# mouzzarr/go-libp2p-pubsub

Measured on AMD Instinct MI355X. Metric: peer-heartbeat updates/sec + msg-edge deliveries/sec, 1M-peer gossipsub sim, higher is better.
Workload: dtype f64; 1 GPU; c3: 1000000 peers, random-regular k=32, one IP per peer, 16 topics, beacon-style params, 4 msg/s/topic, 10 rounds/heartbeat; peers_per_gpu=1000000, degree=32, topics=16, edge_topic_records=512000000, rounds_per_heartbeat=10

## Files before the change

go-libp2p-pubsub_amd/csrc/gsim_internal.h:

```cpp
#pragma once
#include <hip/hip_runtime.h>

#include <cstdint>
#include <string>
#include <vector>

#include "gsim.h"

#include <atomic>
namespace gsim {
extern std::atomic<unsigned long long> g_host_syncs;
inline hipError_t counted_stream_sync(hipStream_t s)
{
    g_host_syncs.fetch_add(1, std::memory_order_relaxed);
    return (hipStreamSynchronize)(s);
}
inline hipError_t counted_memcpy(void* dst, const void* src, size_t n, hipMemcpyKind k)
{
    g_host_syncs.fetch_add(1, std::memory_order_relaxed);
    return (hipMemcpy)(dst, src, n, k);
}
}
#define hipStreamSynchronize(s) ::gsim::counted_stream_sync(s)
#define hipMemcpy(d, s, n, k) ::gsim::counted_memcpy(d, s, n, k)
// ... 80 lines not shown
    return d > 0 ? div_trunc_pos(n, d) : n / d;
}

template <class A>
__device__ __forceinline__ const A& kernarg0(const A& arg)
{
    using CP = const __attribute__((address_space(4))) A*;
    CP p = (CP)__builtin_amdgcn_kernarg_segment_ptr();
    asm volatile("" : "+s"(p));
#ifdef GSIM_DEBUG_KERNARG
    static_assert(sizeof(A) >= 16, "kernarg0 check reads 16 bytes");
    const uint64_t* x = (const uint64_t*)&arg;
    const __attribute__((address_space(4))) uint64_t* y = (const __attribute__((address_space(4))) uint64_t*)p;
    if (x[0] != y[0] || x[1] != y[1]) __builtin_trap();
#else
    (void)arg;
#endif
    return *(const A*)p;
}

__device__ __forceinline__ int64_t lazy_mtime(int32_t lazy, int64_t R, int64_t graft, int64_t stored)
{
    return lazy && graft <= R ? R - graft : stored;
}

__device__ __forceinline__ uint64_t smask_of(const uint64_t* smask, uint32_t owner)
{
    return smask ? smask[owner] : ~0ull;
}
__device__ __forceinline__ bool slot_has(uint64_t m, int32_t t) { return (m >> t) & 1ull; }
__device__ __forceinline__ int64_t slot_idx(uint64_t m, int32_t t, int64_t E, int64_t x)
{
    return (int64_t)__popcll(m & ((1ull << t) - 1ull)) * E + x;
}
__device__ __forceinline__ int32_t slot_topic(uint64_t m, int32_t p)
{
    for (int32_t k = 0; k < p; ++k) m &= m - 1;
    return m ? __builtin_ctzll(m) : -1;
}

typedef const __attribute__((address_space(4))) gsim_topic_score_params* ctp_t;
__device__ __forceinline__ ctp_t const_tp(const gsim_topic_score_params* p)
{
    return (ctp_t)(p);
}

enum FieldKind : int {
    FK_RAW = 0,
    FK_RECORD,
    FK_TRECORD,
    FK_TEDGE,
    FK_TFLAGS,
    FK_ESTATE,
    FK_SEEN,
};

struct FieldRef {
    void* ptr;
    size_t bytes;
    int kind = FK_RAW;
    int elem = 1;
    int npar = 1;
};

struct Deliver;

// ... 411 lines not shown
```

go-libp2p-pubsub_amd/csrc/heartbeat.hip:

```cpp
#include <hip/hip_runtime.h>

#include <algorithm>
#include <vector>

#include "gsim.h"
#include "gsim_internal.h"
#include "philox.h"

using namespace gsim;

constexpr int kGiantRow = 8192;
constexpr int kWideB = 1024;
constexpr int kWideBytes = 64;
#ifndef GSIM_HB_HUBV
#define GSIM_HB_HUBV 2
#endif
#define GSIM_HUB_SCHEME_(s1, s2, s3) (GSIM_HB_HUBV == 1 ? (s1) : GSIM_HB_HUBV == 2 ? (s2) : (s3))
constexpr int kHubB[6] = {GSIM_HUB_SCHEME_(128, 64, 64), GSIM_HUB_SCHEME_(256, 128, 64), GSIM_HUB_SCHEME_(512, 256, 128),
                          GSIM_HUB_SCHEME_(1024, 512, 256), 1024, 1024};
constexpr int kHubVv[6] = {GSIM_HUB_SCHEME_(1, 2, 2), GSIM_HUB_SCHEME_(1, 2, 4), GSIM_HUB_SCHEME_(1, 2, 4),
                           GSIM_HUB_SCHEME_(1, 2, 4), 2, 4};
static_assert(kHubB[0] * kHubVv[0] == 128 && kHubB[1] * kHubVv[1] == 256 && kHubB[2] * kHubVv[2] == 512 &&
              kHubB[3] * kHubVv[3] == 1024 && kHubB[4] * kHubVv[4] == 2048 && kHubB[5] * kHubVv[5] == 4096,
              "a hub class's block covers its longest row");

struct Extra {
    uint8_t* d_ctl = nullptr;
    uint64_t* d_cany = nullptr;
    int64_t* d_lastpub = nullptr;
    uint64_t* d_fantopics = nullptr;
    uint32_t max_degree = 0;
    uint64_t seed = 0x9E3779B97F4A7C15ull;
    uint32_t* d_rows = nullptr;
    int64_t n16 = 0, n32 = 0, n64 = 0;
    int64_t n8 = 0;
// ... 120 lines not shown
    if constexpr (W == 64) {
        return wave_min_u32(v);
    } else {
        static_assert(W == 32 || W == 16 || W == 8, "groups of 8, 16, 32 or 64 lanes");
        const int I = -1;
        v = min(v, (uint32_t)__builtin_amdgcn_update_dpp(I, (int)v, 0x111, 0xF, 0xF, false));
        v = min(v, (uint32_t)__builtin_amdgcn_update_dpp(I, (int)v, 0x112, 0xF, 0xF, false));
        v = min(v, (uint32_t)__builtin_amdgcn_update_dpp(I, (int)v, 0x114, 0xF, 0xF, false));
        if constexpr (W == 8) {
            uint32_t r = 0;
#pragma unroll
            for (int q = 0; q < 8; ++q) {
                const uint32_t x = (uint32_t)__builtin_amdgcn_readlane((int)v, 8 * q + 7);
                if (grp == q) r = x;
            }
            return r;
        }
        v = min(v, (uint32_t)__builtin_amdgcn_update_dpp(I, (int)v, 0x118, 0xF, 0xF, false));
        if constexpr (W == 32) {
            v = min(v, (uint32_t)__builtin_amdgcn_update_dpp(I, (int)v, 0x142, 0xA, 0xF, false));
            const uint32_t lo = (uint32_t)__builtin_amdgcn_readlane((int)v, 31);
            const uint32_t hi = (uint32_t)__builtin_amdgcn_readlane((int)v, 63);
            return grp ? hi : lo;
        } else {
            const uint32_t r0 = (uint32_t)__builtin_amdgcn_readlane((int)v, 15);
            const uint32_t r1 = (uint32_t)__builtin_amdgcn_readlane((int)v, 31);
            const uint32_t r2 = (uint32_t)__builtin_amdgcn_readlane((int)v, 47);
            const uint32_t r3 = (uint32_t)__builtin_amdgcn_readlane((int)v, 63);
            return grp == 0 ? r0 : grp == 1 ? r1 : grp == 2 ? r2 : r3;
        }
    }
}

__device__ __forceinline__ uint32_t glob(const HbArgs& a, uint32_t p) { return a.gid ? a.gid[p] : p; }

__device__ __forceinline__ uint64_t hb_key(const HbArgs& a, uint32_t obs, int32_t t, uint32_t purpose, uint32_t col,
                                           uint32_t pos)
{
    return select_key(a.seed, (uint32_t)a.tick, obs, (uint32_t)t, purpose, col, pos);
}

__device__ __forceinline__ uint32_t hb_key_hi(const HbArgs& a, uint32_t obs, int32_t t, uint32_t purpose,
                                              uint32_t col, uint32_t pos)
{
    return (uint32_t)(select_key(a.seed, (uint32_t)a.tick, obs, (uint32_t)t, purpose, col, pos) >> 32);
}

template <int W = 64>
__device__ bool select_smallest(const HbArgs& a, bool cand, int count, uint32_t obs, int32_t t, uint32_t purpose,
                                uint32_t col, uint32_t pos, uint64_t gm = ~0ull, int grp = 0)
{
    const uint64_t avail = __ballot(cand) & gm;
    const int n = __popcll(avail);
    if (n == 0) return false;
    if (count <= 0 || n <= count) return cand;
    const int lane = threadIdx.x & 63;
    uint32_t hi = 0xFFFFFFFFu;
    if (cand) hi = hb_key_hi(a, obs, t, purpose, col, pos);
    const uint32_t tau = (uint32_t)((float)count / (float)n * 4294967040.0f);
    bool sel = cand && hi < tau;
    int c = __popcll(__ballot(sel) & gm);
    while (c > count) {
        const uint32_t mx = ~group_min_u32<W>(sel ? ~hi : 0xFFFFFFFFu, grp);
        const uint64_t at = __ballot(sel && hi == mx) & gm;
        const int win = 63 - __clzll((long long)at);
        if (lane == win) sel = false;
        --c;
    }
    uint32_t rest = (cand && !sel) ? hi : 0xFFFFFFFFu;
    uint64_t left = __ballot(cand && !sel) & gm;
    while (c < count) {
        const uint32_t mn = group_min_u32<W>(rest, grp);
        const int win = __ffsll((long long)(__ballot(rest == mn) & left)) - 1;
        left &= ~(1ull << win);
        if (lane == win) { sel = true; rest = 0xFFFFFFFFu; }
        ++c;
    }
    return sel;
}

__device__ __forceinline__ const HbArgs& hb_launder(const HbArgs& a)
{
    return kernarg0(a);
}

struct ScoreFlags {
    int64_t ir;
    bool ok = false;
    uint8_t v = 0, v0 = 0;
    bool have = false;
    __device__ void at(uint64_t mj, int32_t t, int64_t E, uint32_t rv)
    {
        ok = slot_has(mj, t);
        ir = slot_idx(mj, t, E, rv);
    }
    __device__ uint8_t& get(const HbArgs& a)
    {
        if (!have) { v = v0 = ok ? a.tflags[ir] : 0; have = true; }
        return v;
    }
    __device__ void store(const HbArgs& a) const
    {
        if (ok && have && v != v0) a.tflags[ir] = v;
    }
};

__device__ __forceinline__ void stats_graft(const HbArgs& a, bool tracked, bool scored, ScoreFlags& sf)
{
    if (!tracked || !scored || !sf.ok) return;
    uint8_t& fl = sf.get(a);
    fl = (uint8_t)((fl | GSIM_TF_IN_MESH) & ~GSIM_TF_ACTIVE);
    a.graft[sf.ir] = a.now;
    a.mtime[sf.ir] = 0;
}

__device__ __forceinline__ void stats_prune(const HbArgs& a, bool tracked, bool scored, double thr, double mcap,
                                            ScoreFlags& sf)
{
    if (!tracked || !scored || !sf.ok) return;
    uint8_t& fl = sf.get(a);
    if (fl & GSIM_TF_ACTIVE) {
        const double md = apply_incs(a.meshd[sf.ir], a.mcnt[sf.ir], mcap);
        if (md < thr) {
            const double deficit = thr - md;
            a.fail[sf.ir] = a.fail[sf.ir] + deficit * deficit;
        }
    }
// ... 48 lines not shown
                                                                       : a.mtime[slot_idx(mj, t, a.E, rv)];
                double p1 = 0.0;
                if (tp->time_in_mesh_quantum_ns != 0) p1 = (double)go_div(mt[j], tp->time_in_mesh_quantum_ns);
                if (p1 > tp->time_in_mesh_cap) p1 = tp->time_in_mesh_cap;
                ts += p1 * tp->time_in_mesh_weight;
            }
            ts += f[j] * tp->first_message_deliveries_weight;
            if (fl[j] & GSIM_TF_ACTIVE) {
                if (meshd < tp->mesh_message_deliveries_threshold) {
                    const double deficit = tp->mesh_message_deliveries_threshold - meshd;
                    const double p3 = deficit * deficit;
                    ts += p3 * tp->mesh_message_deliveries_weight;
                }
            }
            ts += fa[j] * tp->mesh_failure_penalty_weight;
            const double p4 = iv[j] * iv[j];
            ts += p4 * tp->invalid_message_deliveries_weight;
            score += ts * tp->topic_weight;
        }
    }
    if (a.topic_cap > 0 && score > a.topic_cap) score = a.topic_cap;
    score += a.p5[col] * a.w5;
    score += a.p6[rv] * a.w6;
    const double bp = a.bp[rv];
    if (bp > a.bp_thr) {
        const double excess = bp - a.bp_thr;
        const double p7 = excess * excess;
        score += p7 * a.w7;
    }
    return score;
}

template <int W = 64>
__device__ bool gossip_targets(const HbArgs& a, bool cand, bool tpeer, uint32_t obs, int32_t t, uint32_t col,
                               uint32_t pos, uint64_t gm = ~0ull, int grp = 0)
{
    const int c = __popcll(__ballot(cand) & gm);
    bool dup = false;
    if (c < a.Dlo) dup = select_smallest<W>(a, tpeer, a.Dlo - c, obs, t, P_GOSSIP_FILL, col, pos, gm, grp);
    const int n = c + __popcll(__ballot(dup) & gm);
    if (n == 0) return false;
    int target = a.dlazy;
    const int factor = (int)(a.gossip_factor * (double)n);
    if (factor > target) target = factor;
    if (target >= n) return cand || dup;
    if (!(__ballot(dup) & gm)) return select_smallest<W>(a, cand, target, obs, t, P_GOSSIP, col, pos, gm, grp);
    uint32_t h1 = cand ? hb_key_hi(a, obs, t, P_GOSSIP, col, pos) : 0xFFFFFFFFu;
    uint32_t h2 = dup ? hb_key_hi(a, obs, t, P_GOSSIP_DUP, col, pos) : 0xFFFFFFFFu;
    uint64_t av1 = __ballot(cand) & gm, av2 = __ballot(dup) & gm;
    const int lane = threadIdx.x & 63;
    bool sel = false;
    for (int q = 0; q < target; ++q) {
        const bool has1 = (av1 >> lane) & 1ull, has2 = (av2 >> lane) & 1ull;
        const bool use1 = has1 && (!has2 || h1 <= h2);
        const uint32_t mine = use1 ? h1 : (has2 ? h2 : 0xFFFFFFFFu);
        const uint32_t mn = group_min_u32<W>(mine, grp);
        const bool at_min = mine == mn && (has1 || has2);
        const int win = __ffsll((long long)(__ballot(at_min) & gm)) - 1;
        if ((__ballot(at_min && use1) >> win) & 1ull) av1 &= ~(1ull << win); else av2 &= ~(1ull << win);
        if (lane == win) sel = true;
    }
    return sel;
}




template <int W>
struct WaveGroup {
    static constexpr int V = 1;
    static constexpr int LP = 64 / W;
    int lane, grp, gl, base;
    uint64_t gm;
    int32_t lpv[LP];
    __device__ explicit WaveGroup(int lane_)
        : lane(lane_), grp(lane_ / W), gl(lane_ % W), base((lane_ / W) * W),
          gm(W == 64 ? ~0ull : (((1ull << W) - 1) << ((lane_ / W) * W)))
    {
    }
    __device__ int pos(int = 0) const { return gl; }
    __device__ int span() const { return W; }
    __device__ int count(const bool* p) const { return __popcll(__ballot(p[0]) & gm); }
    __device__ bool any(const bool* p) const { return (__ballot(p[0]) & gm) != 0; }
    __device__ void select(const HbArgs& a, const bool* cand, int count, uint32_t obs, int32_t t, uint32_t purpose,
                           const uint32_t* col, bool* out)
    {
        out[0] = select_smallest<W>(a, cand[0], count, obs, t, purpose, col[0], (uint32_t)gl, gm, grp);
    }
    __device__ void gossip(const HbArgs& a, const bool* cand, const bool* tpeer, uint32_t obs, int32_t t,
                           const uint32_t* col, bool* out)
    {
        out[0] = gossip_targets<W>(a, cand[0], tpeer[0], obs, t, col[0], (uint32_t)gl, gm, grp);
    }
    template <typename T>
    struct View {
        T v;
        int base;
        __device__ T operator[](int q) const { return __shfl(v, base + q, 64); }
    };
    struct BoolView {
        uint64_t m;
        int base;
        __device__ bool operator[](int q) const { return (m >> (base + q)) & 1ull; }
    };
    template <int SLOT, typename T>
    __device__ View<T> view(const T* v) const { return View<T>{v[0], base}; }
    template <int SLOT>
    __device__ BoolView view_b(const bool* v) const { return BoolView{__ballot(v[0]), base}; }
    static constexpr bool kList = false;
    __device__ double at_lowest(const bool* p, const double* v) const
    {
        return __shfl(v[0], (int)__ffsll((long long)(__ballot(p[0]) & gm)) - 1, 64);
    }
    __device__ uint64_t topic_mask(bool p) const { return __ballot(p) & gm; }
    static constexpr bool kRowMask = true;
    __device__ uint64_t row_mask(const bool* p) const { return (__ballot(p[0]) & gm) >> base; }
    __device__ void load_lastput(const HbArgs& a, int64_t obs, uint64_t subi, bool ovalid)
    {
#pragma unroll
        for (int k = 0; k < LP; ++k) {
            const int32_t t = gl + W * k;
            lpv[k] = (a.gossip && ovalid && t < a.T && ((subi >> t) & 1ull)) ? a.lastput[(int64_t)t * a.N + obs] : -1;
        }
    }
    __device__ int32_t lastput(const HbArgs&, int64_t, int32_t t) const
    {
        int32_t lpsel = lpv[0];
#pragma unroll
        for (int k = 1; k < LP; ++k)
            if (t >= W * k) lpsel = lpv[k];
        return __shfl(lpsel, base + (t & (W - 1)), 64);
    }
};

template <int B, int VV = 1>
struct BlockGroup {
    static constexpr int V = VV;
    static constexpr int NW = B / 64;
    static constexpr int P = B * V;
    struct Shared {
        unsigned long long red[2][NW];
        double d0[P];
        uint64_t u0[P], u1[P];
        int32_t i0[P];
        int32_t l0[P];
        int ln;
        uint8_t b0[P], b1[P];
    };
    Shared* sh;
    int tid, lane, wid, phase;
    __device__ BlockGroup(Shared* s) : sh(s), tid((int)threadIdx.x), lane((int)threadIdx.x & 63),
                                       wid((int)threadIdx.x >> 6), phase(0) {}
    __device__ int pos(int v = 0) const { return v * B + tid; }
    __device__ int span() const { return P; }
    __device__ unsigned long long reduce(unsigned long long v, int op)
    {
        for (int o = 32; o; o >>= 1) {
            const unsigned long long y = (unsigned long long)__shfl_xor((long long)v, o, 64);
            v = op == 0 ? v + y : op == 1 ? (y < v ? y : v) : (y > v ? y : v);
        }
        unsigned long long* r = sh->red[phase & 1];
        ++phase;
        if (lane == 0) r[wid] = v;
        __syncthreads();
        unsigned long long acc = r[0];
        for (int w = 1; w < NW; ++w) {
            const unsigned long long y = r[w];
            acc = op == 0 ? acc + y : op == 1 ? (y < acc ? y : acc) : (y > acc ? y : acc);
        }
        return acc;
// ... 143 lines not shown
    __device__ double at_lowest(const bool* p, const double* v)
    {
        uint64_t mine = ~0ull;
#pragma unroll
        for (int x = V - 1; x >= 0; --x) if (p[x]) mine = (uint64_t)pos(x);
        const uint64_t q = min_u64(mine);
        __syncthreads();
#pragma unroll
        for (int x = 0; x < V; ++x) if ((uint64_t)pos(x) == q) sh->d0[0] = v[x];
        __syncthreads();
        return sh->d0[0];
    }
    static constexpr bool kRowMask = false;
    __device__ uint64_t row_mask(const bool*) const { return 0; }
    __device__ uint64_t topic_mask(bool p)
    {
        const uint64_t m = __ballot(p);
        return reduce((wid == 0 && lane == 0) ? m : 0ull, 0);
    }
    __device__ void load_lastput(const HbArgs&, int64_t, uint64_t, bool) {}
    __device__ int32_t lastput(const HbArgs& a, int64_t obs, int32_t t) const
    {
        return a.lastput[(int64_t)t * a.N + obs];
    }
};

}

template <class Grp>
__device__ __forceinline__ void hb_observer(const HbArgs& a_, Grp& g, int64_t obs, bool ovalid)
{
        const HbArgs& a = a_;
        constexpr int V = Grp::V;
        const uint32_t b = ovalid ? a.row_ptr[obs] : 0u;
        const int deg = ovalid ? (int)(a.row_ptr[obs + 1] - b) : 0;
        const uint32_t gobs = ovalid ? glob(a, (uint32_t)obs) : 0u;
        const uint64_t subi = ovalid ? a.sub[obs] : 0ull;
        const uint64_t mi = ovalid ? smask_of(a.smask, (uint32_t)obs) : 0ull;
        int gl[V];
        bool valid[V], tracked[V], conn[V], outb[V], dir[V], dirty[V];
        uint32_t e[V], col[V], rv[V], gcol[V];
        double S[V], S_live[V];
        uint64_t subj[V], mj[V];
#pragma unroll
        for (int v = 0; v < V; ++v) {
            gl[v] = g.pos(v);
            valid[v] = gl[v] < deg;
            e[v] = b + (uint32_t)gl[v];
            col[v] = valid[v] ? a.col[e[v]] : 0u;
            rv[v] = valid[v] ? a.rev[e[v]] : 0u;
            gcol[v] = valid[v] ? glob(a, col[v]) : 0u;
            const uint8_t est = valid[v] ? a.estate[rv[v]] : 0;
            tracked[v] = est & GSIM_ES_TRACKED;
            conn[v] = valid[v] && (a.rstate[e[v]] & GSIM_ES_CONNECTED);
            outb[v] = valid[v] && a.outbound[e[v]];
            dir[v] = valid[v] && a.direct[e[v]];
            S[v] = valid[v] ? a.score[rv[v]] : 0.0;
            subj[v] = !valid[v] ? 0ull : a.sub_all ? ~0ull : a.sub[col[v]];
            mj[v] = valid[v] ? smask_of(a.smask, col[v]) : 0ull;
            S_live[v] = S[v];
            dirty[v] = false;
            if (a.gossip && valid[v]) a.gstate[e[v]] = S[v] >= a.gossip_thr ? 1 : 0;
        }
        g.load_lastput(a, obs, subi, ovalid);
        uint64_t pxt = 0;
        auto rescore = [&]() {
            if (g.any(dirty)) {
#pragma unroll
                for (int v = 0; v < V; ++v) {
                    if (dirty[v]) S_live[v] = score_of_record(a, rv[v], col[v]);
                    dirty[v] = false;
                }
            }
        };

        if (a.tick % 15 == 0) {
#pragma unroll
            for (int v = 0; v < V; ++v) {
                if (!valid[v]) continue;
                for (int32_t t = 0; t < a.T; ++t) {
                    if (!slot_has(mi, t)) continue;
                    const int64_t i = slot_idx(mi, t, a.E, e[v]);
                    const int64_t bo = a.backoff[i];
                    if (bo != 0 && bo + kBackoffSlack < a.now) a.backoff[i] = 0;
                }
            }
        }

        for (int32_t t0 = 0; t0 < a.T; t0 += kFlagChunk) {
          if (!((subi >> t0) & ((1ull << kFlagChunk) - 1))) continue;
          uint8_t flc[kFlagChunk][V];
#pragma unroll
          for (int j = 0; j < kFlagChunk; ++j) {
              const int32_t t = t0 + j;
#pragma unroll
              for (int v = 0; v < V; ++v)
                  flc[j][v] = (t < a.T && valid[v] && ((subi >> t) & 1ull)) ? a.mflags[slot_idx(mi, t, a.E, e[v])] : 0;
          }
          for (int j = 0; j < kFlagChunk; ++j) {
            const int32_t t = t0 + j;
            if (t >= a.T) break;
            if (!((subi >> t) & 1ull)) continue;
            const HbArgs& a = hb_launder(a_);
            const ctp_t tp = const_tp(a.tp) + t;
            const bool scored = tp->scored != 0;
            const double thr = tp->mesh_message_deliveries_threshold;
            const double mcap = tp->mesh_message_deliveries_cap;
            int64_t i[V];
            ScoreFlags sf[V];
            uint8_t fl[V], fl0[V], ctl[V];
            int64_t bo[V];
            bool have_bo[V], bo_dirty[V], tpeer[V], m[V], cand[V], sel[V];
#pragma unroll
            for (int v = 0; v < V; ++v) {
                i[v] = slot_idx(mi, t, a.E, e[v]);
                sf[v].at(mj[v], t, a.E, rv[v]);
                fl[v] = flc[j][v];
                fl0[v] = fl[v];
                bo[v] = 0;
                have_bo[v] = bo_dirty[v] = false;
                tpeer[v] = valid[v] && conn[v] && ((subj[v] >> t) & 1ull);
                m[v] = valid[v] && (fl[v] & GSIM_TF_MESH);
                ctl[v] = 0;
            }
            auto need_bo = [&](int v) {
                if (!have_bo[v]) {
#ifdef GSIM_DIAG_HB
                    if (valid[v]) atomicAdd(&g_hb_diag[3], 1ull);
#endif
                    bo[v] = valid[v] ? a.backoff[i[v]] : 0;
                    have_bo[v] = true;
                }
            };
            auto prune = [&](int v) {
#ifdef GSIM_DIAG_HB
                atomicAdd(&g_hb_diag[2], 1ull);
#endif
                if (a.tr.on((uint32_t)obs)) a.tr.push(a.now, 0, (uint32_t)obs, col[v], t, GSIM_TRACE_PRUNE, 0);
                stats_prune(a, tracked[v], scored, thr, mcap, sf[v]);
                dirty[v] |= tracked[v] && scored;
                fl[v] &= (uint8_t)~GSIM_TF_MESH;
                m[v] = false;
                need_bo(v);
                const int64_t ex = a.now + a.prune_backoff;
                if (bo[v] < ex) { bo[v] = ex; bo_dirty[v] = true; }
                ctl[v] |= GSIM_CTL_PRUNE;
            };
            auto graft = [&](int v) {
#ifdef GSIM_DIAG_HB
                atomicAdd(&g_hb_diag[1], 1ull);
#endif
                if (a.tr.on((uint32_t)obs)) a.tr.push(a.now, 0, (uint32_t)obs, col[v], t, GSIM_TRACE_GRAFT, 0);
                stats_graft(a, tracked[v], scored, sf[v]);
                dirty[v] |= tracked[v] && scored;
                fl[v] |= GSIM_TF_MESH;
                m[v] = true;
// ... 123 lines not shown
                    }
                    const int jj = a.Dout - obD < nb ? a.Dout - obD : nb;
#pragma unroll
                    for (int v = 0; v < V; ++v) keep[v] = (inD[v] && !(rest[v] && rr[v] < jj)) || (cb[v] && rb[v] < jj);
                }
#pragma unroll
                for (int v = 0; v < V; ++v)
                    if (m[v] && !keep[v]) {
                        prune(v);
                        if (a.do_px) ctl[v] |= GSIM_CTL_PX;
                    }
            }

            l = g.count(m);
            if (l >= a.Dlo) {
                bool mo[V];
#pragma unroll
                for (int v = 0; v < V; ++v) mo[v] = m[v] && outb[v];
                const int ob = g.count(mo);
                if (ob < a.Dout) {
#pragma unroll
                    for (int v = 0; v < V; ++v) {
                        need_bo(v);
                        cand[v] = tpeer[v] && !m[v] && bo[v] == 0 && !dir[v] && outb[v] && S[v] >= 0;
                    }
                    g.select(a, cand, a.Dout - ob, gobs, t, P_GRAFT_DOUT, gcol, sel);
#pragma unroll
                    for (int v = 0; v < V; ++v)
                        if (sel[v]) graft(v);
                }
            }

            l = g.count(m);
            if (a.opp_ticks && a.tick % a.opp_ticks == 0 && l > 1) {
                int rank[V];
#pragma unroll
                for (int v = 0; v < V; ++v) rank[v] = 0;
                {
                    const auto vm = g.template view_b<0>(m);
                    const auto vs = g.template view<0>(S);
                    if constexpr (Grp::kList) {
                        g.each(m, [&](int q) {
                            const double sq = vs[q];
                            const bool mq = vm[q];
#pragma unroll
                            for (int v = 0; v < V; ++v)
                                if (mq && (sq < S[v] || (sq == S[v] && q < gl[v]))) ++rank[v];
                        });
                    } else {
                        for (int q = 0; q < g.span(); ++q) {
                            const double sq = vs[q];
                            const bool mq = vm[q];
#pragma unroll
                            for (int v = 0; v < V; ++v)
                                if (mq && (sq < S[v] || (sq == S[v] && q < gl[v]))) ++rank[v];
                        }
                    }
                }
                bool atm[V];
#pragma unroll
                for (int v = 0; v < V; ++v) atm[v] = m[v] && rank[v] == l / 2;
                const double median = g.at_lowest(atm, S);
                if (median < a.opp_threshold) {
#pragma unroll
                    for (int v = 0; v < V; ++v) {
                        need_bo(v);
                        cand[v] = tpeer[v] && !m[v] && bo[v] == 0 && !dir[v] && S[v] > median;
                    }
                    g.select(a, cand, a.opp_peers, gobs, t, P_GRAFT_OPP, gcol, sel);
#pragma unroll
                    for (int v = 0; v < V; ++v)
                        if (sel[v]) graft(v);
                }
            }

#pragma unroll
            for (int v = 0; v < V; ++v) {
                if (!valid[v]) continue;
                if (fl[v] != fl0[v]) a.mflags[i[v]] = fl[v];
                sf[v].store(a);
                if (bo_dirty[v]) a.backoff[i[v]] = bo[v];
            }
          {
            const HbArgs& a = hb_launder(a_);
            if constexpr (Grp::kRowMask) {
                if (a.mmask) {
                    bool mm[V];
#pragma unroll
                    for (int v = 0; v < V; ++v)
                        mm[v] = valid[v] && (m[v] || dir[v]) && col[v] >= a.mlo && col[v] < a.mhi;
                    const uint64_t mk = g.row_mask(mm);
                    if (gl[0] == 0 && ovalid) a.mmask[(int64_t)t * a.N + obs] = mk;
                }
            }

            if (a.gossip) {
                bool gs[V];
#pragma unroll
                for (int v = 0; v < V; ++v) gs[v] = false;
                const int32_t lpt = g.lastput(a, obs, t);
                if (lpt >= 0 && lpt >= (int64_t)a.tick - a.hist_gossip) {
                    rescore();
#pragma unroll
                    for (int v = 0; v < V; ++v)
                        cand[v] = tpeer[v] && !m[v] && !dir[v] && S_live[v] >= a.gossip_thr;
                    g.gossip(a, cand, tpeer, gobs, t, gcol, gs);
                }
#pragma unroll
                for (int v = 0; v < V; ++v)
                    if (valid[v]) a.gsel[i[v]] = gs[v] ? 1 : 0;
            }
            bool pxc[V];
#pragma unroll
            for (int v = 0; v < V; ++v) {
                if (valid[v] && ctl[v] && slot_has(mj[v], t)) {
                    const int64_t r = slot_idx(mj[v], t, a.E, rv[v]);
                    a.ctl_out[r] = (uint8_t)(a.ctl_out[r] | ctl[v]);
                    atomicOr(reinterpret_cast<unsigned long long*>(a.cany_out + col[v]), 1ull << t);
                }
                pxc[v] = (ctl[v] & GSIM_CTL_PX) != 0;
            }
            if (a.do_px && g.any(pxc)) pxt |= 1ull << t;
          }
          }
        }
        if (a.do_px && pxt) {
            rescore();
#pragma unroll
            for (int v = 0; v < V; ++v)
                if (valid[v]) a.pxs[e[v]] = S_live[v];
            if (gl[0] == 0 && ovalid) a.pxo[obs] = pxt;
        }
}

template <int W>
#ifndef GSIM_HB_WPE
#define GSIM_HB_WPE 5
#endif
#ifndef GSIM_HB_WPE16
#define GSIM_HB_WPE16 4
#endif
#ifndef GSIM_CHURN_MCNT
#define GSIM_CHURN_MCNT 1
#endif
#ifndef GSIM_HB_W8
#define GSIM_HB_W8 1
#endif
__global__ __launch_bounds__(256) __attribute__((amdgpu_waves_per_eu(W <= 16 ? GSIM_HB_WPE16 : GSIM_HB_WPE)))
void k_heartbeat(HbArgs a, const uint32_t* rows, int64_t nrows, int64_t obs_base)
{
    constexpr int G = 64 / W;
    const int lane = threadIdx.x & 63, wid = threadIdx.x >> 6;
    WaveGroup<W> g(lane);
    for (int64_t o0 = ((int64_t)blockIdx.x * 4 + wid) * G; o0 < nrows; o0 += (int64_t)gridDim.x * 4 * G) {
        const bool ovalid = o0 + g.grp < nrows;
        const int64_t obs = !ovalid ? 0 : rows ? (int64_t)rows[o0 + g.grp] : obs_base + o0 + g.grp;
        hb_observer(a, g, obs, ovalid);
    }
}

template <int B, int V>
__global__ __launch_bounds__(B) void k_heartbeat_hub(HbArgs a, const uint32_t* rows, int64_t nrows)
{
    __shared__ typename BlockGroup<B, V>::Shared sh;
    BlockGroup<B, V> g(&sh);
    for (int64_t o = blockIdx.x; o < nrows; o += gridDim.x) hb_observer(a, g, (int64_t)rows[o], true);
}

template <int B, int V>
__global__ __launch_bounds__(B) void k_heartbeat_hub_g(HbArgs a, const uint32_t* rows, int64_t nrows, void* scratch)
{
    using S = typename BlockGroup<B, V>::Shared;
    BlockGroup<B, V> g(reinterpret_cast<S*>(scratch) + blockIdx.x);
    for (int64_t o = blockIdx.x; o < nrows; o += gridDim.x) hb_observer(a, g, (int64_t)rows[o], true);
}

template <class Grp>
__device__ __forceinline__ void fanout_observer(const HbArgs& a, Grp& g, int64_t obs)
{
        constexpr int V = Grp::V;
        const int gl0 = g.pos(0);
        const int64_t lpub = gl0 < a.T ? a.lastpub[obs * a.T + gl0] : 0;
        const uint64_t expired = g.topic_mask(lpub != 0 && lpub + a.fanout_ttl < a.now);
        const uint64_t fant0 = a.fan_topics[obs];
        if (!expired && !fant0) return;
        const uint32_t b = a.row_ptr[obs];
// ... 1320 lines not shown
                           1024u);
    if (h->x->nh8192)
        hipLaunchKernelGGL((k_fanout_publish_hub_g<1024, kGiantRow / 1024>),
                           dim3((uint32_t)std::min<int64_t>(count, h->x->gscratch_blocks)), dim3(1024), 0, h->stream, a,
                           d_pub, count, 4096u, h->x->d_gscratch);
    if (h->x->nwide) launch_fanout_publish_wide(h, a, d_pub, count);
    return hip_check(h, hipGetLastError(), "k_fanout_publish");
}

extern "C" {

int gsim_set_seed(gsim_handle* h, uint64_t seed)
{
    if (!h || !h->x) return GSIM_EINVAL;
    h->x->seed = seed;
    return GSIM_OK;
}

int gsim_heartbeat(gsim_handle* h, uint64_t tick, int64_t now)
{
    if (!h) return GSIM_EINVAL;
    if (hipSetDevice(h->device) != hipSuccess) return GSIM_EDEVICE;
    if (h->e == 0 || !h->x) { h->err = "no graph loaded"; return GSIM_ESTATE; }
    int rc = GSIM_OK;
    if (!h->in_step) rc = deliver_check_errors(h);
    if (rc) return rc;
    rc = deliver_flush(h);
    if (!rc) rc = deliver_heartbeat_begin(h, tick);
    if (rc) return rc;
    HbArgs a = make_hb_args(h, tick, now, 1);
    ProfScope ps(h, GSIM_K_HEARTBEAT);
    const Extra* x = h->x;
    const int64_t nown = h->ohi() - h->olo();
    if (x->n16 == nown && !x->d_rows) {
        hipLaunchKernelGGL(k_heartbeat<16>, dim3(grid_rows((nown + 3) / 4)), dim3(256), 0, h->stream, a, nullptr, nown,
                           h->olo());
    } else if (x->n32 == nown && !x->d_rows) {
        hipLaunchKernelGGL(k_heartbeat<32>, dim3(grid_rows((nown + 1) / 2)), dim3(256), 0, h->stream, a, nullptr, nown,
                           h->olo());
    } else if (x->n64 == nown && !x->d_rows) {
        hipLaunchKernelGGL(k_heartbeat<64>, dim3(grid_rows(nown)), dim3(256), 0, h->stream, a, nullptr, nown, h->olo());
    } else {
        const uint32_t* r = x->d_rows;
        if (x->n8) hipLaunchKernelGGL(k_heartbeat<8>, dim3(grid_rows((x->n8 + 7) / 8)), dim3(256), 0, h->stream,
                                      a, r, x->n8, (int64_t)0);
        if (x->n16 > x->n8)
            hipLaunchKernelGGL(k_heartbeat<16>, dim3(grid_rows((x->n16 - x->n8 + 3) / 4)), dim3(256), 0, h->stream,
                               a, r + x->n8, x->n16 - x->n8, (int64_t)0);
        if (x->n32) hipLaunchKernelGGL(k_heartbeat<32>, dim3(grid_rows((x->n32 + 1) / 2)), dim3(256), 0, h->stream,
                                       a, r + x->n16, x->n32, (int64_t)0);
        if (x->n64) hipLaunchKernelGGL(k_heartbeat<64>, dim3(grid_rows(x->n64)), dim3(256), 0, h->stream,
                                       a, r + x->n16 + x->n32, x->n64, (int64_t)0);
        const uint32_t* rh = r + x->n16 + x->n32 + x->n64;
        auto hub = [&](auto kern, int bt, int64_t off, int64_t n) {
            if (n > 0)
                hipLaunchKernelGGL(kern, dim3((uint32_t)std::min<int64_t>(n, 65536)), dim3(bt), 0, h->stream, a, rh + off, n);
        };
        hub(k_heartbeat_hub<kHubB[0], kHubVv[0]>, kHubB[0], 0, x->nh128);
        hub(k_heartbeat_hub<kHubB[1], kHubVv[1]>, kHubB[1], x->nh128, x->nh256 - x->nh128);
        hub(k_heartbeat_hub<kHubB[2], kHubVv[2]>, kHubB[2], x->nh256, x->nh512);
        hub(k_heartbeat_hub<kHubB[3], kHubVv[3]>, kHubB[3], x->nh256 + x->nh512, x->nh1024 - x->nh512);
        hub(k_heartbeat_hub<kHubB[4], kHubVv[4]>, kHubB[4], x->nh256 + x->nh1024, x->nh2048);
        hub(k_heartbeat_hub<kHubB[5], kHubVv[5]>, kHubB[5], x->nh256 + x->nh1024 + x->nh2048, x->nh4096 - x->nh2048);
        if (x->nh8192)
            hipLaunchKernelGGL((k_heartbeat_hub_g<1024, kGiantRow / 1024>), dim3((uint32_t)x->gscratch_blocks), dim3(1024),
                               0, h->stream, a, rh + x->nh256 + x->nh1024 + x->nh4096, x->nh8192, x->d_gscratch);
        if (x->nwide) launch_heartbeat_wide(h, a);
    }
    hipLaunchKernelGGL(k_fanout_heartbeat, dim3(grid_rows(nown)), dim3(256), 0, h->stream, a);
    const uint32_t* rh = x->d_rows + x->n16 + x->n32 + x->n64;
    if (x->nh256)
        hipLaunchKernelGGL((k_fanout_heartbeat_hub<256, 1>), dim3((uint32_t)std::min<int64_t>(x->nh256, 65536)),
                           dim3(256), 0, h->stream, a, rh, x->nh256);
    if (x->nh1024)
        hipLaunchKernelGGL((k_fanout_heartbeat_hub<1024, 1>), dim3((uint32_t)std::min<int64_t>(x->nh1024, 65536)),
                           dim3(1024), 0, h->stream, a, rh + x->nh256, x->nh1024);
    if (x->nh4096)
        hipLaunchKernelGGL((k_fanout_heartbeat_hub<1024, 4>), dim3((uint32_t)std::min<int64_t>(x->nh4096, 65536)),
                           dim3(1024), 0, h->stream, a, rh + x->nh256 + x->nh1024, x->nh4096);
    if (x->nh8192)
        hipLaunchKernelGGL((k_fanout_heartbeat_hub_g<1024, kGiantRow / 1024>), dim3((uint32_t)x->gscratch_blocks),
                           dim3(1024), 0, h->stream, a, rh + x->nh256 + x->nh1024 + x->nh4096, x->nh8192, x->d_gscratch);
    if (x->nwide) launch_fanout_heartbeat_wide(h, a);
    if (a.do_px)
        launch_px_emit(h, a, 1, (uint32_t)tick, (uint32_t)P_PX);
// ... 262 lines not shown
        hipLaunchKernelGGL(k_px_pairs, dim3((n + 255) / 256), dim3(256), 0, h->stream, (const uint32_t*)pxc, n,
                           (const uint32_t*)h->d_owner, (const uint32_t*)h->d_col, pxc + 1 + 2 * (size_t)n);
        std::vector<uint32_t> pv(2 * (size_t)n);
        e = hipGetLastError();
        if (e == hipSuccess)
            e = hipMemcpyAsync(pv.data(), pxc + 1 + 2 * (size_t)n, sizeof(uint32_t) * pv.size(), hipMemcpyDeviceToHost,
                               h->stream);
        if (e == hipSuccess) e = hipStreamSynchronize(h->stream);
        if (e != hipSuccess) return hip_check(h, e, "gsim_px_connect pairs");
        std::vector<std::pair<uint32_t, uint32_t>> pr((size_t)n);
        for (size_t q = 0; q < n; ++q) pr[q] = {pv[2 * q], pv[2 * q + 1]};
        std::sort(pr.begin(), pr.end());
        for (size_t q = 0; q < n && (int64_t)q < cap; ++q) { pairs[2 * q] = pr[q].first; pairs[2 * q + 1] = pr[q].second; }
    }
    int rc = deliver_flush(h);
    if (!rc && !GSIM_CHURN_MCNT) rc = materialize_mcnt(h);
    if (rc) return rc;
    ProfScope ps(h, GSIM_K_CHURN);
    hipLaunchKernelGGL(k_px_outbound, dim3((n + 255) / 256), dim3(256), 0, h->stream, (const uint32_t*)pxc, n,
                       h->d_outbound);
    e = hipGetLastError();
    if (e != hipSuccess) return hip_check(h, e, "k_px_outbound");
    return apply_connections(h, pxc + 1, (int32_t)(2 * n), 1, now);
}

}

#ifdef GSIM_DIAG_HB
extern "C" int gsim_diag_hb_counts(gsim_handle* h, uint64_t* out4)
{
    if (!h || !out4) return GSIM_EINVAL;
    if (hipStreamSynchronize(h->stream) != hipSuccess) return GSIM_EDEVICE;
    unsigned long long z[4] = {0, 0, 0, 0};
    if (hipMemcpyFromSymbol(out4, HIP_SYMBOL(g_hb_diag), sizeof(z)) != hipSuccess) return GSIM_EDEVICE;
    if (hipMemcpyToSymbol(HIP_SYMBOL(g_hb_diag), z, sizeof(z)) != hipSuccess) return GSIM_EDEVICE;
    return GSIM_OK;
}
#endif


namespace {

enum : uint8_t {
    WB_M = 1,
    WB_TPEER = 2,
    WB_HAVE_BO = 4,
    WB_BO_DIRTY = 8,
    WB_SF_HAVE = 16,
    WB_CAND = 32,
    WB_SEL = 64,
    WB_DIRTY = 128
};
enum : uint8_t { WC_DUP = 1, WC_HAS1 = 2, WC_HAS2 = 4, WC_GS = 8, WC_REST = 16 };
enum : uint8_t { WL_OUTB = 1, WL_TAIL = 2, WL_REST = 4, WL_CB = 8 };

struct WideRow {
    struct Shared {
        unsigned long long red[2][kWideB / 64];
        int ln;
        double d;
    };
    double *S, *Sl;
    double* lS;
    uint64_t* key;
    uint64_t* lk;
    int64_t* bo;
    int32_t *lq, *lp;
    uint8_t *fl, *fl0, *ctl, *sfv, *sfv0, *bits, *bits2, *lb;
// ... 642 lines not shown
```

Before: 22.77 million peer-heartbeat updates/sec.

## Skip mesh maintenance for steady lane-group rows and specialize dense topic slots

Adds a wave-level steady-state test in the lane-group heartbeat path. When every row's mesh size is within [Dlo, Dhi], the outbound quota is met, no mesh peer has a negative score, and it is not an opportunistic-graft tick, the per-topic maintenance (score flags, backoff, graft/prune selection, control output) is skipped. It also adds a Dense template variant, used when there is no subscription mask, that computes slot indices directly instead of with popcount. Group ballots are narrowed to 32-bit group bits and the float division becomes a reciprocal. The risk is a behaviour change if skipped maintenance had side effects the steady test does not cover, such as score-flag or backoff updates.

```diff
diff --git a/go-libp2p-pubsub_amd/csrc/gsim_internal.h b/go-libp2p-pubsub_amd/csrc/gsim_internal.h
--- a/go-libp2p-pubsub_amd/csrc/gsim_internal.h
+++ b/go-libp2p-pubsub_amd/csrc/gsim_internal.h
@@ -136,6 +136,16 @@
 __device__ __forceinline__ int64_t slot_idx(uint64_t m, int32_t t, int64_t E, int64_t x)
 {
     return (int64_t)__popcll(m & ((1ull << t) - 1ull)) * E + x;
+}
+template <bool Dense>
+__device__ __forceinline__ bool slot_has_of(uint64_t m, int32_t t)
+{
+    if constexpr (Dense) return true; else return slot_has(m, t);
+}
+template <bool Dense>
+__device__ __forceinline__ int64_t slot_idx_of(uint64_t m, int32_t t, int64_t E, int64_t x)
+{
+    if constexpr (Dense) return (int64_t)t * E + x; else return slot_idx(m, t, E, x);
 }
 __device__ __forceinline__ int32_t slot_topic(uint64_t m, int32_t p)
 {
diff --git a/go-libp2p-pubsub_amd/csrc/heartbeat.hip b/go-libp2p-pubsub_amd/csrc/heartbeat.hip
--- a/go-libp2p-pubsub_amd/csrc/heartbeat.hip
+++ b/go-libp2p-pubsub_amd/csrc/heartbeat.hip
@@ -1,6 +1,7 @@
 #include <hip/hip_runtime.h>
 
 #include <algorithm>
+#include <type_traits>
 #include <vector>
 
 #include "gsim.h"
@@ -187,6 +188,37 @@
     }
 }
 
+template <int W>
+struct GroupBits {
+    static_assert(W == 64 || W == 32 || W == 16 || W == 8, "groups of 8, 16, 32 or 64 lanes");
+    using bits_t = std::conditional_t<W == 64, uint64_t, uint32_t>;
+    int grp;
+    __device__ explicit GroupBits(int grp_) : grp(grp_) {}
+    __device__ bits_t of(uint64_t bal) const
+    {
+        if constexpr (W == 64) {
+            return bal;
+        } else {
+            constexpr int H = 32 / W;
+            const uint32_t half = grp >= H ? (uint32_t)(bal >> 32) : (uint32_t)bal;
+            if constexpr (W == 32) return half;
+            else return (half >> ((grp & (H - 1)) * W)) & ((1u << W) - 1u);
+        }
+    }
+    __device__ static int popc(bits_t x)
+    {
+        if constexpr (W == 64) return __popcll(x); else return __popc(x);
+    }
+    __device__ static int lowest(bits_t x)
+    {
+        if constexpr (W == 64) return __ffsll((long long)x) - 1; else return __ffs((int)x) - 1;
+    }
+    __device__ static int highest(bits_t x)
+    {
+        if constexpr (W == 64) return 63 - __clzll((long long)x); else return 31 - __clz((int)x);
+    }
+};
+
 __device__ __forceinline__ uint32_t glob(const HbArgs& a, uint32_t p) { return a.gid ? a.gid[p] : p; }
 
 __device__ __forceinline__ uint64_t hb_key(const HbArgs& a, uint32_t obs, int32_t t, uint32_t purpose, uint32_t col,
@@ -201,35 +233,48 @@
     return (uint32_t)(select_key(a.seed, (uint32_t)a.tick, obs, (uint32_t)t, purpose, col, pos) >> 32);
 }
 
+#if GSIM_DIAG_HB == 2
+__device__ unsigned long long g_hb_sel[4];
+#endif
+
 template <int W = 64>
 __device__ bool select_smallest(const HbArgs& a, bool cand, int count, uint32_t obs, int32_t t, uint32_t purpose,
-                                uint32_t col, uint32_t pos, uint64_t gm = ~0ull, int grp = 0)
-{
-    const uint64_t avail = __ballot(cand) & gm;
-    const int n = __popcll(avail);
+                                uint32_t col, uint32_t pos, int grp = 0)
+{
+    using GB = GroupBits<W>;
+    const GB gb(grp);
+    const int n = GB::popc(gb.of(__ballot(cand)));
     if (n == 0) return false;
     if (count <= 0 || n <= count) return cand;
-    const int lane = threadIdx.x & 63;
+    const int gl = (int)(threadIdx.x & (W - 1));
     uint32_t hi = 0xFFFFFFFFu;
     if (cand) hi = hb_key_hi(a, obs, t, purpose, col, pos);
-    const uint32_t tau = (uint32_t)((float)count / (float)n * 4294967040.0f);
+    const uint32_t tau = (uint32_t)((float)count * __builtin_amdgcn_rcpf((float)n) * 4294967040.0f);
     bool sel = cand && hi < tau;
-    int c = __popcll(__ballot(sel) & gm);
+    int c = GB::popc(gb.of(__ballot(sel)));
+#if GSIM_DIAG_HB == 2
+    if (gl == 0) atomicAdd(&g_hb_sel[0], 1ull);
+#endif
     while (c > count) {
         const uint32_t mx = ~group_min_u32<W>(sel ? ~hi : 0xFFFFFFFFu, grp);
-        const uint64_t at = __ballot(sel && hi == mx) & gm;
-        const int win = 63 - __clzll((long long)at);
-        if (lane == win) sel = false;
+        const int win = GB::highest(gb.of(__ballot(sel && hi == mx)));
+        if (gl == win) sel = false;
         --c;
+#if GSIM_DIAG_HB == 2
+        if (gl == 0) atomicAdd(&g_hb_sel[1], 1ull);
+#endif
     }
     uint32_t rest = (cand && !sel) ? hi : 0xFFFFFFFFu;
-    uint64_t left = __ballot(cand && !sel) & gm;
+    typename GB::bits_t left = gb.of(__ballot(cand && !sel));
     while (c < count) {
         const uint32_t mn = group_min_u32<W>(rest, grp);
-        const int win = __ffsll((long long)(__ballot(rest == mn) & left)) - 1;
-        left &= ~(1ull << win);
-        if (lane == win) { sel = true; rest = 0xFFFFFFFFu; }
+        const int win = GB::lowest(gb.of(__ballot(rest == mn)) & left);
+        left &= ~((typename GB::bits_t)1 << win);
+        if (gl == win) { sel = true; rest = 0xFFFFFFFFu; }
         ++c;
+#if GSIM_DIAG_HB == 2
+        if (gl == 0) atomicAdd(&g_hb_sel[2], 1ull);
+#endif
     }
     return sel;
 }
@@ -237,6 +282,11 @@
 __device__ __forceinline__ const HbArgs& hb_launder(const HbArgs& a)
 {
     return kernarg0(a);
+}
+template <bool Again>
+__device__ __forceinline__ const HbArgs& hb_launder_if(const HbArgs& a, const HbArgs& cur)
+{
+    if constexpr (Again) return hb_launder(a); else return cur;
 }
 
 struct ScoreFlags {
@@ -244,10 +294,11 @@
     bool ok = false;
     uint8_t v = 0, v0 = 0;
     bool have = false;
+    template <bool Dense = false>
     __device__ void at(uint64_t mj, int32_t t, int64_t E, uint32_t rv)
     {
-        ok = slot_has(mj, t);
-        ir = slot_idx(mj, t, E, rv);
+        ok = slot_has_of<Dense>(mj, t);
+        ir = slot_idx_of<Dense>(mj, t, E, rv);
     }
     __device__ uint8_t& get(const HbArgs& a)
     {
@@ -362,33 +413,37 @@
 }
 
 template <int W = 64>
-__device__ bool gossip_targets(const HbArgs& a, bool cand, bool tpeer, uint32_t obs, int32_t t, uint32_t col,
-                               uint32_t pos, uint64_t gm = ~0ull, int grp = 0)
-{
-    const int c = __popcll(__ballot(cand) & gm);
+__device__ __forceinline__ bool gossip_targets(const HbArgs& a, bool cand, bool tpeer, uint32_t obs, int32_t t, uint32_t col,
+                               uint32_t pos, int grp = 0)
+{
+    using GB = GroupBits<W>;
+    using bits_t = typename GB::bits_t;
+    const GB gb(grp);
+    const int c = GB::popc(gb.of(__ballot(cand)));
     bool dup = false;
-    if (c < a.Dlo) dup = select_smallest<W>(a, tpeer, a.Dlo - c, obs, t, P_GOSSIP_FILL, col, pos, gm, grp);
-    const int n = c + __popcll(__ballot(dup) & gm);
+    if (c < a.Dlo) dup = select_smallest<W>(a, tpeer, a.Dlo - c, obs, t, P_GOSSIP_FILL, col, pos, grp);
+    bits_t av2 = gb.of(__ballot(dup));
+    const int n = c + GB::popc(av2);
     if (n == 0) return false;
     int target = a.dlazy;
     const int factor = (int)(a.gossip_factor * (double)n);
     if (factor > target) target = factor;
     if (target >= n) return cand || dup;
-    if (!(__ballot(dup) & gm)) return select_smallest<W>(a, cand, target, obs, t, P_GOSSIP, col, pos, gm, grp);
+    if (!av2) return select_smallest<W>(a, cand, target, obs, t, P_GOSSIP, col, pos, grp);
     uint32_t h1 = cand ? hb_key_hi(a, obs, t, P_GOSSIP, col, pos) : 0xFFFFFFFFu;
     uint32_t h2 = dup ? hb_key_hi(a, obs, t, P_GOSSIP_DUP, col, pos) : 0xFFFFFFFFu;
-    uint64_t av1 = __ballot(cand) & gm, av2 = __ballot(dup) & gm;
-    const int lane = threadIdx.x & 63;
+    bits_t av1 = gb.of(__ballot(cand));
+    const int gl = (int)(threadIdx.x & (W - 1));
     bool sel = false;
     for (int q = 0; q < target; ++q) {
-        const bool has1 = (av1 >> lane) & 1ull, has2 = (av2 >> lane) & 1ull;
+        const bool has1 = (av1 >> gl) & 1, has2 = (av2 >> gl) & 1;
         const bool use1 = has1 && (!has2 || h1 <= h2);
         const uint32_t mine = use1 ? h1 : (has2 ? h2 : 0xFFFFFFFFu);
         const uint32_t mn = group_min_u32<W>(mine, grp);
         const bool at_min = mine == mn && (has1 || has2);
-        const int win = __ffsll((long long)(__ballot(at_min) & gm)) - 1;
-        if ((__ballot(at_min && use1) >> win) & 1ull) av1 &= ~(1ull << win); else av2 &= ~(1ull << win);
-        if (lane == win) sel = true;
+        const int win = GB::lowest(gb.of(__ballot(at_min)));
+        if ((gb.of(__ballot(at_min && use1)) >> win) & 1) av1 &= ~((bits_t)1 << win); else av2 &= ~((bits_t)1 << win);
+        if (gl == win) sel = true;
     }
     return sel;
 }
@@ -396,13 +451,15 @@
 
 
 
-template <int W>
+template <int W, bool Dense_ = false>
 struct WaveGroup {
     static constexpr int V = 1;
+    static constexpr bool kDense = Dense_;
     static constexpr int LP = 64 / W;
     int lane, grp, gl, base;
     uint64_t gm;
     int32_t lpv[LP];
+    bool opp_tick = false;
     __device__ explicit WaveGroup(int lane_)
         : lane(lane_), grp(lane_ / W), gl(lane_ % W), base((lane_ / W) * W),
           gm(W == 64 ? ~0ull : (((1ull << W) - 1) << ((lane_ / W) * W)))
@@ -410,17 +467,39 @@
     }
     __device__ int pos(int = 0) const { return gl; }
     __device__ int span() const { return W; }
-    __device__ int count(const bool* p) const { return __popcll(__ballot(p[0]) & gm); }
-    __device__ bool any(const bool* p) const { return (__ballot(p[0]) & gm) != 0; }
+    __device__ typename GroupBits<W>::bits_t bits(bool p) const { return GroupBits<W>(grp).of(__ballot(p)); }
+    __device__ int count(const bool* p) const { return GroupBits<W>::popc(bits(p[0])); }
+    __device__ bool any(const bool* p) const { return bits(p[0]) != 0; }
+    static constexpr bool kSteadyTest = true;
+    __device__ bool steady(bool m, bool mo, bool neg, int Dlo, int Dhi, int Dout) const
+    {
+        if (__ballot(neg)) return false;
+        if constexpr (W >= 32) {
+            const uint64_t bm = __ballot(m), bo = __ballot(mo), ex = __ballot(true);
+            bool ok = true;
+#pragma unroll
+            for (int h = 0; h < 64 / W; ++h) {
+                constexpr uint64_t gmask = W == 64 ? ~0ull : 0xFFFFFFFFull;
+                const int sh = W == 64 ? 0 : h * W;
+                if (!((ex >> sh) & gmask)) continue;
+                const int l = __popcll((bm >> sh) & gmask), ob = __popcll((bo >> sh) & gmask);
+                ok = ok && l >= Dlo && l <= Dhi && ob >= Dout;
+            }
+            return ok;
+        } else {
+            const int l = GroupBits<W>::popc(bits(m)), ob = GroupBits<W>::popc(bits(mo));
+            return !__ballot(l < Dlo || l > Dhi || ob < Dout);
+        }
+    }
     __device__ void select(const HbArgs& a, const bool* cand, int count, uint32_t obs, int32_t t, uint32_t purpose,
                            const uint32_t* col, bool* out)
     {
-        out[0] = select_smallest<W>(a, cand[0], count, obs, t, purpose, col[0], (uint32_t)gl, gm, grp);
+        out[0] = select_smallest<W>(a, cand[0], count, obs, t, purpose, col[0], (uint32_t)gl, grp);
     }
     __device__ void gossip(const HbArgs& a, const bool* cand, const bool* tpeer, uint32_t obs, int32_t t,
                            const uint32_t* col, bool* out)
     {
-        out[0] = gossip_targets<W>(a, cand[0], tpeer[0], obs, t, col[0], (uint32_t)gl, gm, grp);
+        out[0] = gossip_targets<W>(a, cand[0], tpeer[0], obs, t, col[0], (uint32_t)gl, grp);
     }
     template <typename T>
     struct View {
@@ -440,11 +519,11 @@
     static constexpr bool kList = false;
     __device__ double at_lowest(const bool* p, const double* v) const
     {
-        return __shfl(v[0], (int)__ffsll((long long)(__ballot(p[0]) & gm)) - 1, 64);
+        return __shfl(v[0], base + GroupBits<W>::lowest(bits(p[0])), 64);
     }
     __device__ uint64_t topic_mask(bool p) const { return __ballot(p) & gm; }
     static constexpr bool kRowMask = true;
-    __device__ uint64_t row_mask(const bool* p) const { return (__ballot(p[0]) & gm) >> base; }
+    __device__ uint64_t row_mask(const bool* p) const { return bits(p[0]); }
     __device__ void load_lastput(const HbArgs& a, int64_t obs, uint64_t subi, bool ovalid)
     {
 #pragma unroll
@@ -466,6 +545,9 @@
 template <int B, int VV = 1>
 struct BlockGroup {
     static constexpr int V = VV;
+    static constexpr bool kDense = false;
+    static constexpr bool kSteadyTest = false;
+    static constexpr bool opp_tick = false;
     static constexpr int NW = B / 64;
     static constexpr int P = B * V;
     struct Shared {
@@ -675,6 +757,7 @@
 {
         const HbArgs& a = a_;
         constexpr int V = Grp::V;
+        constexpr bool kDense = Grp::kDense;
         const uint32_t b = ovalid ? a.row_ptr[obs] : 0u;
         const int deg = ovalid ? (int)(a.row_ptr[obs + 1] - b) : 0;
         const uint32_t gobs = ovalid ? glob(a, (uint32_t)obs) : 0u;
@@ -722,8 +805,8 @@
             for (int v = 0; v < V; ++v) {
                 if (!valid[v]) continue;
                 for (int32_t t = 0; t < a.T; ++t) {
-                    if (!slot_has(mi, t)) continue;
-                    const int64_t i = slot_idx(mi, t, a.E, e[v]);
+                    if (!slot_has_of<kDense>(mi, t)) continue;
+                    const int64_t i = slot_idx_of<kDense>(mi, t, a.E, e[v]);
                     const int64_t bo = a.backoff[i];
                     if (bo != 0 && bo + kBackoffSlack < a.now) a.backoff[i] = 0;
                 }
@@ -738,33 +821,59 @@
               const int32_t t = t0 + j;
 #pragma unroll
               for (int v = 0; v < V; ++v)
-                  flc[j][v] = (t < a.T && valid[v] && ((subi >> t) & 1ull)) ? a.mflags[slot_idx(mi, t, a.E, e[v])] : 0;
+                  flc[j][v] = (t < a.T && valid[v] && ((subi >> t) & 1ull)) ? a.mflags[slot_idx_of<kDense>(mi, t, a.E, e[v])] : 0;
           }
           for (int j = 0; j < kFlagChunk; ++j) {
             const int32_t t = t0 + j;
             if (t >= a.T) break;
             if (!((subi >> t) & 1ull)) continue;
-            const HbArgs& a = hb_launder(a_);
-            const ctp_t tp = const_tp(a.tp) + t;
-            const bool scored = tp->scored != 0;
-            const double thr = tp->mesh_message_deliveries_threshold;
-            const double mcap = tp->mesh_message_deliveries_cap;
+            constexpr bool kSteady = Grp::kSteadyTest;
             int64_t i[V];
             ScoreFlags sf[V];
             uint8_t fl[V], fl0[V], ctl[V];
             int64_t bo[V];
-            bool have_bo[V], bo_dirty[V], tpeer[V], m[V], cand[V], sel[V];
+            bool have_bo[V], bo_dirty[V], tpeer[V], m[V], cand[V];
+            bool scored = false;
+            double thr = 0.0, mcap = 0.0;
+            auto topic_params = [&](const HbArgs& a) {
+                const ctp_t tp = const_tp(a.tp) + t;
+                scored = tp->scored != 0;
+                thr = tp->mesh_message_deliveries_threshold;
+                mcap = tp->mesh_message_deliveries_cap;
+            };
+            const HbArgs& a0 = hb_launder(a_);
+            if constexpr (!kSteady) topic_params(a0);
 #pragma unroll
             for (int v = 0; v < V; ++v) {
-                i[v] = slot_idx(mi, t, a.E, e[v]);
-                sf[v].at(mj[v], t, a.E, rv[v]);
+                i[v] = slot_idx_of<kDense>(mi, t, a0.E, e[v]);
+                if constexpr (!kSteady) sf[v].template at<kDense>(mj[v], t, a0.E, rv[v]);
                 fl[v] = flc[j][v];
                 fl0[v] = fl[v];
-                bo[v] = 0;
-                have_bo[v] = bo_dirty[v] = false;
+                if constexpr (!kSteady) { bo[v] = 0; have_bo[v] = bo_dirty[v] = false; }
                 tpeer[v] = valid[v] && conn[v] && ((subj[v] >> t) & 1ull);
                 m[v] = valid[v] && (fl[v] & GSIM_TF_MESH);
                 ctl[v] = 0;
+            }
+            bool maintain = true;
+            if constexpr (kSteady) {
+                static_assert(V == 1, "lane groups hold one row position per lane");
+                maintain = g.opp_tick ||
+                           !g.steady(m[0], m[0] && outb[0], m[0] && S[0] < 0, a0.Dlo, a0.Dhi, a0.Dout);
+            }
+            if (maintain) {
+#if GSIM_DIAG_HB == 2
+            if constexpr (kSteady) if (__ffsll((long long)__ballot(true)) - 1 == (int)(threadIdx.x & 63)) atomicAdd(&g_hb_sel[3], 1ull);
+#endif
+            const HbArgs& a = hb_launder_if<kSteady>(a_, a0);
+            bool sel[V];
+            if constexpr (kSteady) {
+                topic_params(a);
+#pragma unroll
+                for (int v = 0; v < V; ++v) {
+                    sf[v].template at<kDense>(mj[v], t, a.E, rv[v]);
+                    bo[v] = 0;
+                    have_bo[v] = bo_dirty[v] = false;
+                }
             }
             auto need_bo = [&](int v) {
                 if (!have_bo[v]) {
@@ -954,7 +1063,7 @@
             }
 
             l = g.count(m);
-            if (a.opp_ticks && a.tick % a.opp_ticks == 0 && l > 1) {
+            if ((kSteady ? g.opp_tick : (a.opp_ticks && a.tick % a.opp_ticks == 0)) && l > 1) {
                 int rank[V];
 #pragma unroll
                 for (int v = 0; v < V; ++v) rank[v] = 0;
@@ -1003,6 +1112,7 @@
                 sf[v].store(a);
                 if (bo_dirty[v]) a.backoff[i[v]] = bo[v];
             }
+            }
           {
             const HbArgs& a = hb_launder(a_);
             if constexpr (Grp::kRowMask) {
@@ -1032,17 +1142,19 @@
                 for (int v = 0; v < V; ++v)
                     if (valid[v]) a.gsel[i[v]] = gs[v] ? 1 : 0;
             }
+            if (maintain) {
             bool pxc[V];
 #pragma unroll
             for (int v = 0; v < V; ++v) {
-                if (valid[v] && ctl[v] && slot_has(mj[v], t)) {
-                    const int64_t r = slot_idx(mj[v], t, a.E, rv[v]);
+                if (valid[v] && ctl[v] && slot_has_of<kDense>(mj[v], t)) {
+                    const int64_t r = slot_idx_of<kDense>(mj[v], t, a.E, rv[v]);
                     a.ctl_out[r] = (uint8_t)(a.ctl_out[r] | ctl[v]);
                     atomicOr(reinterpret_cast<unsigned long long*>(a.cany_out + col[v]), 1ull << t);
                 }
                 pxc[v] = (ctl[v] & GSIM_CTL_PX) != 0;
             }
             if (a.do_px && g.any(pxc)) pxt |= 1ull << t;
+            }
           }
           }
         }
@@ -1055,7 +1167,7 @@
         }
 }
 
-template <int W>
+template <int W, bool Dense>
 #ifndef GSIM_HB_WPE
 #define GSIM_HB_WPE 5
 #endif
@@ -1073,7 +1185,8 @@
 {
     constexpr int G = 64 / W;
     const int lane = threadIdx.x & 63, wid = threadIdx.x >> 6;
-    WaveGroup<W> g(lane);
+    WaveGroup<W, Dense> g(lane);
+    g.opp_tick = a.opp_ticks && a.tick % a.opp_ticks == 0;
     for (int64_t o0 = ((int64_t)blockIdx.x * 4 + wid) * G; o0 < nrows; o0 += (int64_t)gridDim.x * 4 * G) {
         const bool ovalid = o0 + g.grp < nrows;
         const int64_t obs = !ovalid ? 0 : rows ? (int64_t)rows[o0 + g.grp] : obs_base + o0 + g.grp;
@@ -2460,25 +2573,25 @@
     ProfScope ps(h, GSIM_K_HEARTBEAT);
     const Extra* x = h->x;
     const int64_t nown = h->ohi() - h->olo();
+    auto lanes = [&](auto w, const uint32_t* r, int64_t n, int64_t base) {
+        constexpr int W = decltype(w)::value;
+        const dim3 grid(grid_rows((n + 64 / W - 1) / (64 / W)));
+        if (a.smask) hipLaunchKernelGGL((k_heartbeat<W, false>), grid, dim3(256), 0, h->stream, a, r, n, base);
+        else hipLaunchKernelGGL((k_heartbeat<W, true>), grid, dim3(256), 0, h->stream, a, r, n, base);
+    };
+    using std::integral_constant;
     if (x->n16 == nown && !x->d_rows) {
-        hipLaunchKernelGGL(k_heartbeat<16>, dim3(grid_rows((nown + 3) / 4)), dim3(256), 0, h->stream, a, nullptr, nown,
-                           h->olo());
+        lanes(integral_constant<int, 16>{}, nullptr, nown, h->olo());
     } else if (x->n32 == nown && !x->d_rows) {
-        hipLaunchKernelGGL(k_heartbeat<32>, dim3(grid_rows((nown + 1) / 2)), dim3(256), 0, h->stream, a, nullptr, nown,
-                           h->olo());
+        lanes(integral_constant<int, 32>{}, nullptr, nown, h->olo());
     } else if (x->n64 == nown && !x->d_rows) {
-        hipLaunchKernelGGL(k_heartbeat<64>, dim3(grid_rows(nown)), dim3(256), 0, h->stream, a, nullptr, nown, h->olo());
+        lanes(integral_constant<int, 64>{}, nullptr, nown, h->olo());
     } else {
         const uint32_t* r = x->d_rows;
-        if (x->n8) hipLaunchKernelGGL(k_heartbeat<8>, dim3(grid_rows((x->n8 + 7) / 8)), dim3(256), 0, h->stream,
-                                      a, r, x->n8, (int64_t)0);
-        if (x->n16 > x->n8)
-            hipLaunchKernelGGL(k_heartbeat<16>, dim3(grid_rows((x->n16 - x->n8 + 3) / 4)), dim3(256), 0, h->stream,
-                               a, r + x->n8, x->n16 - x->n8, (int64_t)0);
-        if (x->n32) hipLaunchKernelGGL(k_heartbeat<32>, dim3(grid_rows((x->n32 + 1) / 2)), dim3(256), 0, h->stream,
-                                       a, r + x->n16, x->n32, (int64_t)0);
-        if (x->n64) hipLaunchKernelGGL(k_heartbeat<64>, dim3(grid_rows(x->n64)), dim3(256), 0, h->stream,
-                                       a, r + x->n16 + x->n32, x->n64, (int64_t)0);
+        if (x->n8) lanes(integral_constant<int, 8>{}, r, x->n8, 0);
+        if (x->n16 > x->n8) lanes(integral_constant<int, 16>{}, r + x->n8, x->n16 - x->n8, 0);
+        if (x->n32) lanes(integral_constant<int, 32>{}, r + x->n16, x->n32, 0);
+        if (x->n64) lanes(integral_constant<int, 64>{}, r + x->n16 + x->n32, x->n64, 0);
         const uint32_t* rh = r + x->n16 + x->n32 + x->n64;
         auto hub = [&](auto kern, int bt, int64_t off, int64_t n) {
             if (n > 0)
@@ -2807,8 +2920,13 @@
     if (!h || !out4) return GSIM_EINVAL;
     if (hipStreamSynchronize(h->stream) != hipSuccess) return GSIM_EDEVICE;
     unsigned long long z[4] = {0, 0, 0, 0};
+#if GSIM_DIAG_HB == 2
+    if (hipMemcpyFromSymbol(out4, HIP_SYMBOL(g_hb_sel), sizeof(z)) != hipSuccess) return GSIM_EDEVICE;
+    if (hipMemcpyToSymbol(HIP_SYMBOL(g_hb_sel), z, sizeof(z)) != hipSuccess) return GSIM_EDEVICE;
+#else
     if (hipMemcpyFromSymbol(out4, HIP_SYMBOL(g_hb_diag), sizeof(z)) != hipSuccess) return GSIM_EDEVICE;
     if (hipMemcpyToSymbol(HIP_SYMBOL(g_hb_diag), z, sizeof(z)) != hipSuccess) return GSIM_EDEVICE;
+#endif
     return GSIM_OK;
 }
 #endif
```

Measured after the change: 23.33 million peer-heartbeat updates/sec (median of 6 runs). 1.02x the previous value.
